# zfountas/deep-active-inference-mc

Measured on AMD Instinct MI355X. Metric: EFE rollouts/sec (64x64 dSprites, 10 MC-samples, depth 5), higher is better.
Workload: dtype f32; 1 GPU; calculate_G_repeated: 128 rows (32 roots x 4 actions) x depth 5 x 10 MC samples per GPU (BASELINE configs[1]) + action posterior; rows_per_gpu=128, samples=10, depth=5, parallelism=episodes sharded x1, weights replicated

## Files before the change

deep-active-inference-mc_amd/build.py:

```python
import hashlib
import os
import subprocess
import sys

HERE = os.path.dirname(os.path.abspath(__file__))
SOURCES = ['csrc/kernels.hip', 'csrc/decoder.hip', 'csrc/encoder.hip', 'csrc/mcts.hip', 'csrc/fused.hip', 'csrc/generic.hip', 'csrc/generic_dec.hip', 'csrc/generic_enc.hip', 'csrc/bf16x3.hip', 'csrc/loss.hip', 'csrc/engine.hip']
HEADERS = ['csrc/kernels.h', 'csrc/philox.h', 'csrc/mfma_pipe.h', 'csrc/ctx_registry.h', '../include/efe_engine.h']
LIB = os.path.join(HERE, 'libefe_mi355x.so')
OPS_SOURCES = ['csrc/torch_ops.cpp']
OPS_LIB = os.path.join(HERE, 'libefe_torch_ops.so')
FLAGS = ['--offload-arch=gfx950', '-O3', '-std=c++17', '-shared', '-fPIC', '-Wno-pass-failed', '-Wl,-soname,libefe_mi355x.so']


def source_digest(files=None):
    h = hashlib.sha256()
    for f in (files or SOURCES + HEADERS):
        path = os.path.join(HERE, f)
        if not os.path.exists(path):
            continue
        h.update(f.encode())
        with open(path, 'rb') as fh:
            h.update(fh.read())
    h.update(' '.join(FLAGS).encode())
    return h.hexdigest()[:16]


def _stamp(lib, marker):
    if not os.path.exists(lib):
        return None
    try:
        data = open(lib, 'rb').read()
        key = (marker + '=').encode()
        i = data.find(key)
        return data[i + len(key):i + len(key) + 16].decode() if i >= 0 else None
    except Exception:
        return None


def needs_build():
    return _stamp(LIB, 'EFE_BUILD_ID') != source_digest()


def _compile_objects(hipcc, srcs, verbose):
    from concurrent.futures import ThreadPoolExecutor
    obj_dir = os.path.join(HERE, 'build')
    os.makedirs(obj_dir, exist_ok=True)
    hdr = source_digest(HEADERS)

    def one(src):
        h = hashlib.sha256(open(src, 'rb').read() + hdr.encode() + ' '.join(FLAGS).encode()).hexdigest()[:16]
        obj = os.path.join(obj_dir, os.path.basename(src) + '.' + h + '.o')
        if not os.path.exists(obj):
            for old in os.listdir(obj_dir):
                if old.startswith(os.path.basename(src) + '.'):
                    os.unlink(os.path.join(obj_dir, old))
            cmd = [hipcc, *[f for f in FLAGS if f != '-shared' and not f.startswith('-Wl,')], '-c', src, '-o', obj]
            if verbose:
                print(' '.join(cmd), flush=True)
            r = subprocess.run(cmd, capture_output=True, text=True)
            if r.returncode != 0:
                sys.stderr.write(r.stdout + r.stderr)
                raise RuntimeError(f'hipcc failed compiling {src}')
        return obj
    with ThreadPoolExecutor(max_workers=min(8, len(srcs))) as ex:
        return list(ex.map(one, srcs))


def build(force=False, verbose=False):
    if force or needs_build():
        hipcc = os.environ.get('HIPCC', '/opt/rocm/bin/hipcc')
        srcs = [os.path.join(HERE, s) for s in SOURCES if os.path.exists(os.path.join(HERE, s))]
        if force:
            import shutil
            shutil.rmtree(os.path.join(HERE, 'build'), ignore_errors=True)
        objs = _compile_objects(hipcc, srcs, verbose)
        stamp = os.path.join(HERE, 'build', 'build_id.cpp')
        with open(stamp, 'w') as fh:
            fh.write('extern "C" const char* efe_build_id(void) {\n'
                     f'    static const char stamp[] = "EFE_BUILD_ID={source_digest()}";      // the marker lets build.py read the stamp from the file without dlopen\n'
                     '    return stamp + 13;\n}\n')
        stamp_o = stamp[:-4] + '.o'
        r = subprocess.run(['g++', '-O1', '-fPIC', '-c', stamp, '-o', stamp_o], capture_output=True, text=True)
        if r.returncode != 0:
            sys.stderr.write(r.stdout + r.stderr)
            raise RuntimeError('g++ failed compiling the build-id stamp')
        cmd = [hipcc, *FLAGS, stamp_o, *objs, '-o', LIB]
        if verbose:
            print(' '.join(cmd))
        r = subprocess.run(cmd, capture_output=True, text=True)
        if r.returncode != 0:
            sys.stderr.write(r.stdout + r.stderr)
            raise RuntimeError('hipcc failed linking libefe_mi355x.so')
    build_torch_ops(force=force, verbose=verbose)
    return LIB


def ops_digest():
    return source_digest(OPS_SOURCES + ['../include/efe_engine.h'])


def build_torch_ops(force=False, verbose=False):
    src = os.path.join(HERE, OPS_SOURCES[0])
    if not os.path.exists(src):
        return None
    if not force and _stamp(OPS_LIB, 'EFE_OPS_BUILD_ID') == ops_digest():
        return OPS_LIB
    import torch
    from torch.utils import cpp_extension as ce
    inc = [f'-I{p}' for p in ce.include_paths()] + ['-I/opt/rocm/include', f'-I{os.path.join(HERE, "..", "include")}']
    tlib = os.path.join(os.path.dirname(torch.__file__), 'lib')
    abi = int(getattr(torch._C, '_GLIBCXX_USE_CXX11_ABI', 1))
    cmd = ['g++', '-O2', '-std=c++17', '-shared', '-fPIC', '-D__HIP_PLATFORM_AMD__=1', '-DUSE_ROCM=1', f'-D_GLIBCXX_USE_CXX11_ABI={abi}',
           f'-DEFE_OPS_BUILD_ID="{ops_digest()}"', *inc, src, '-o', OPS_LIB,
           f'-L{HERE}', '-lefe_mi355x', f'-L{tlib}', '-ltorch', '-ltorch_cpu', '-lc10', '-ltorch_hip', '-lc10_hip',
           '-L/opt/rocm/lib', '-lamdhip64', '-Wl,-rpath,$ORIGIN', f'-Wl,-rpath,{tlib}', '-Wl,-rpath,/opt/rocm/lib']
    if verbose:
        print(' '.join(cmd))
    r = subprocess.run(cmd, capture_output=True, text=True)
    if r.returncode != 0:
        sys.stderr.write(r.stdout + r.stderr)
        raise RuntimeError('g++ failed building libefe_torch_ops.so')
    return OPS_LIB


if __name__ == '__main__':
    print(build(force='--force' in sys.argv, verbose=True))
```

deep-active-inference-mc_amd/csrc/decoder.hip:

```cpp
#include <utility>
#include "mfma_pipe.h"

namespace efe {

template <class F, int... I> __device__ __forceinline__ void static_for_(F&& f, std::integer_sequence<int, I...>) { (f(std::integral_constant<int, I>{}), ...); }
template <int N, class F> __device__ __forceinline__ void static_for(F&& f) { static_for_(f, std::make_integer_sequence<int, N>{}); }

__host__ __device__ constexpr int w3_nch(int G) { return G == 4 ? 5 : 4; }
__host__ __device__ constexpr int w3_prod(int G, int c) {
    return G < 4 ? 5 * ((G >> 1) + 2 * (c >> 1)) + (G & 1) + 2 * (c & 1)
         : G == 4 ? (c < 2 ? 5 * (1 + 2 * c) + 4 : c < 4 ? 20 + 1 + 2 * (c - 2) : 24)
                  : (c < 2 ? 5 * (2 * c) + 4 : 20 + 2 * (c - 2));
}
__host__ __device__ constexpr bool w3_direct(int pp) { return f22_o1(pp / 5) < 0 && f22_o1(pp % 5) < 0; }
__host__ __device__ constexpr int w3_view(int pp) { return 3 * f22_view(pp / 5) + f22_view(pp % 5); }
__host__ __device__ constexpr int w3_mat(int pp) { return 4 * f22_wt(pp / 5) + f22_wt(pp % 5); }
__host__ __device__ constexpr bool w3_hits(int pp, int o) {
    const int r = o >> 2, c = o & 3, pr = pp / 5, pc = pp % 5;
    return (r == f22_o0(pr) || r == f22_o1(pr)) && (c == f22_o0(pc) || c == f22_o1(pc));
}
__host__ __device__ constexpr bool w3_seen(int G, int c, int o) {
    for (int g = 0; g < G; ++g)
        for (int k = 0; k < w3_nch(g); ++k) if (w3_hits(w3_prod(g, k), o)) return true;
    if (!w3_direct(w3_prod(G, c)))
        for (int k = 0; k < w3_nch(G); ++k)
            if ((w3_direct(w3_prod(G, k)) || k < c) && w3_hits(w3_prod(G, k), o)) return true;
    return false;
}
__host__ __device__ constexpr bool w3_uses_view(int G, int vi) {
    for (int k = 0; k < w3_nch(G); ++k) if (w3_view(w3_prod(G, k)) == vi) return true;
    return false;
}
__host__ __device__ constexpr bool f22_in(int a, int r) { return a == 0 ? r <= 1 : (a == 1 ? r == 1 : r >= 1); }
__host__ __device__ constexpr bool w3_reads(int G, int r, int c) {
    for (int vi = 0; vi < 9; ++vi) if (w3_uses_view(G, vi) && f22_in(vi / 3, r) && f22_in(vi % 3, c)) return true;
    return false;
}

constexpr int DA_PS = 17;
constexpr int DA_BIAS = 273 * DA_PS;

__host__ __device__ constexpr int wino_i0(int a) { return a == 0 ? 0 : (a == 2 ? 2 : 1); }
__host__ __device__ constexpr int wino_i1(int a) { return a == 0 ? 2 : (a == 1 ? 2 : (a == 2 ? 1 : 3)); }
__host__ __device__ constexpr float wino_s1(int a) { return a == 1 ? 1.0f : -1.0f; }
__host__ __device__ constexpr float wino_at(int r, int a) { return r == 0 ? (a < 3 ? 1.0f : 0.0f) : (a == 0 ? 0.0f : (a == 1 ? 1.0f : -1.0f)); }

template <int NR, int R0, class Pix>
__device__ __forceinline__ void wino_l1(f32x16 (&out)[NR][2], const float4* __restrict__ U, const float4* sm, const int h,
                                        const int mt_, Pix pix) {
    constexpr int PD = 4;
    const unsigned ln = (threadIdx.x & 63u) * 16u;
    const __amdgpu_buffer_rsrc_t ur = wrsrc(U);
    int mt = mt_; asm volatile("" : "+s"(mt));
    constexpr int a_lo = NR == 2 ? 0 : R0, a_hi = NR == 2 ? 4 : R0 + 3;
    auto ufrag = [&](int a, int b, int kc) { return wfrag(ur, ln, (size_t)(((4 * a + b) * 2 + mt) * 8 + kc) * 64); };
    auto bases = [&](int a, int b, int (&pb)[4]) {
        const int i0 = wino_i0(a), i1 = wino_i1(a), j0 = wino_i0(b), j1 = wino_i1(b);
        pb[0] = pix(i0, j0); pb[1] = pix(i0, j1); pb[2] = pix(i1, j0); pb[3] = pix(i1, j1);
    };
    float4 aq[PD], raw[4];
    int pb[4];
#pragma unroll
    for (int p = 0; p < PD; ++p) aq[p] = ufrag(a_lo, 0, p);
    bases(a_lo, 0, pb);
#pragma unroll
    for (int q = 0; q < 4; ++q) raw[q] = sm[pb[q] + h];
    f32x16 xacc;
    const f32x16 zero = {};
    auto otrans = [&](int a, int b, const f32x16& m, auto mask) {
        constexpr int MASK = decltype(mask)::value;
#pragma unroll
        for (int r = 0; r < NR; ++r) {
            if (!((MASK >> r) & 1)) continue;
            const float car = wino_at(R0 + r, a);
#pragma unroll
            for (int c = 0; c < 2; ++c) {
                const float cbc = wino_at(c, b);
                if (cbc == 0.0f) continue;
                const float cf = car * cbc;
#pragma unroll
                for (int e = 0; e < 16; ++e) out[r][c][e] = __builtin_fmaf(cf, m[e], out[r][c][e]);
            }
        }
    };
    auto xi_row = [&](int a, auto mask) {
        const float s1 = wino_s1(a);
        const int an = a + 1 < a_hi ? a + 1 : a;
#pragma unroll
        for (int b = 0; b < 4; ++b) {
            const float t1 = wino_s1(b);
#pragma unroll
            for (int kc = 0; kc < 8; ++kc) {
                const float4 av = aq[kc % PD];
                aq[kc % PD] = (b * 8 + kc + PD < 32) ? ufrag(a, (b * 8 + kc + PD) >> 3, (kc + PD) & 7) : ufrag(an, 0, (kc + PD) & 7);
                float4 v;
                {
                    const float4 c0 = make_float4(__builtin_fmaf(s1, raw[2].x, raw[0].x), __builtin_fmaf(s1, raw[2].y, raw[0].y),
                                                  __builtin_fmaf(s1, raw[2].z, raw[0].z), __builtin_fmaf(s1, raw[2].w, raw[0].w));
                    const float4 c1 = make_float4(__builtin_fmaf(s1, raw[3].x, raw[1].x), __builtin_fmaf(s1, raw[3].y, raw[1].y),
                                                  __builtin_fmaf(s1, raw[3].z, raw[1].z), __builtin_fmaf(s1, raw[3].w, raw[1].w));
                    v = make_float4(__builtin_fmaf(t1, c1.x, c0.x), __builtin_fmaf(t1, c1.y, c0.y), __builtin_fmaf(t1, c1.z, c0.z), __builtin_fmaf(t1, c1.w, c0.w));
                }
                if (kc < 7) {
#pragma unroll
                    for (int q = 0; q < 4; ++q) raw[q] = sm[pb[q] + 2 * (kc + 1) + h];
                } else {
                    if (b < 3) bases(a, b + 1, pb);
                    else bases(an, 0, pb);
#pragma unroll
                    for (int q = 0; q < 4; ++q) raw[q] = sm[pb[q] + h];
                }
                __builtin_amdgcn_sched_barrier(0);
                f32x16& x = xacc;
                x = __builtin_amdgcn_mfma_f32_32x32x2f32(av.x, v.x, kc == 0 ? zero : x, 0, 0, 0);
                x = __builtin_amdgcn_mfma_f32_32x32x2f32(av.y, v.y, x, 0, 0, 0);
                x = __builtin_amdgcn_mfma_f32_32x32x2f32(av.z, v.z, x, 0, 0, 0);
                x = __builtin_amdgcn_mfma_f32_32x32x2f32(av.w, v.w, x, 0, 0, 0);
            }
            otrans(a, b, xacc, mask);
        }
    };
    if constexpr (NR == 2) {
        xi_row(0, std::integral_constant<int, 1>{});
#pragma unroll 1
        for (int a = 1; a < 3; ++a) xi_row(a, std::integral_constant<int, 3>{});
        xi_row(3, std::integral_constant<int, 2>{});
    } else {
#pragma unroll 1
        for (int a = a_lo; a < a_hi; ++a) xi_row(a, std::integral_constant<int, 1>{});
    }
}
struct F22Nb { int xb, c2[3], r2; };
__device__ __forceinline__ f32x4 f22_wfrag(const __amdgpu_buffer_rsrc_t wr, const unsigned ln, int ct, int m, int kc) {
    return __builtin_bit_cast(f32x4, wfrag(wr, ln + (unsigned)kc * 1024u, (size_t)(m * 4 + ct) * 256));
}
constexpr int F22_PD = 2;
__device__ __forceinline__ void f22_l2_first(f32x4 (&aq)[F22_PD][5], const __amdgpu_buffer_rsrc_t wr, const int dn, const unsigned ln) {
    static_for<F22_PD>([&](auto p) {
        static_for<w3_nch(p >> 2)>([&](auto c) { aq[p][c] = f22_wfrag(wr, ln, dn, w3_mat(w3_prod(p >> 2, c)), p & 3); });
    });
}
__device__ __forceinline__ void f22_l2(f32x4 (&acc)[16], f32x4 (&aq)[F22_PD][5], const __amdgpu_buffer_rsrc_t wr, const int dn,
                                       const unsigned ln, const f32x4 bias4, const f32x4* smv, const F22Nb& nb) {
    constexpr int NST = 24;
    auto px = [&](int i, int jj, int kc) -> f32x4 {
        return smv[(jj == 2 ? nb.c2[i] : (i == 2 ? nb.r2 + jj * DA_PS : nb.xb + (16 * i + jj) * DA_PS)) + 4 * kc];
    };
    auto view = [&](const f32x4 (&x)[9], int vi) -> f32x4 {
        const int va = vi / 3, vb = vi % 3;
        auto cv = [&](int i) -> f32x4 { return vb == 0 ? x[3 * i] - x[3 * i + 1] : (vb == 1 ? x[3 * i + 1] : x[3 * i + 2] - x[3 * i + 1]); };
        return va == 0 ? cv(0) - cv(1) : (va == 1 ? cv(1) : cv(2) - cv(1));
    };
    const f32x4 zero4 = {};
    f32x4 tq[5], xr[9];
    static_for<9>([&](auto i) { if constexpr (w3_reads(0, i / 3, i % 3)) xr[i] = px(i / 3, i % 3, 0); });
    static_for<NST>([&](auto stc) {
        constexpr int ST = decltype(stc)::value, G = ST >> 2, KC = ST & 3, GN = (ST + 1) >> 2, KN = (ST + 1) & 3;
        constexpr int SP = (ST + F22_PD) % NST, GP = SP >> 2, KP = SP & 3;
        f32x4 vw[9], ac[5];
        static_for<9>([&](auto vi) { if constexpr (w3_uses_view(G, vi)) vw[vi] = view(xr, vi); });
#pragma unroll
        for (int c = 0; c < 5; ++c) ac[c] = aq[ST % F22_PD][c];
        static_for<w3_nch(GP)>([&](auto c) { aq[ST % F22_PD][c] = f22_wfrag(wr, ln, ST + F22_PD < NST ? 0 : dn, w3_mat(w3_prod(GP, c)), KP); });
        if constexpr (ST + 1 < NST)
            static_for<9>([&](auto i) { if constexpr (w3_reads(GN, i / 3, i % 3)) xr[i] = px(i / 3, i % 3, KN); });
        __builtin_amdgcn_sched_barrier(0);
#pragma unroll
        for (int e = 0; e < 4; ++e)
            static_for<w3_nch(G)>([&](auto c) {
                constexpr int PP = w3_prod(G, c);
                const float b = vw[w3_view(PP)][e], av = ac[c][e];
                if constexpr (w3_direct(PP)) {
                    constexpr int O = 4 * f22_o0(PP / 5) + f22_o0(PP % 5);
                    constexpr bool FIRST = KC == 0 && !w3_seen(G, c, O);
                    acc[O] = __builtin_amdgcn_mfma_f32_16x16x4f32(av, b, (FIRST && e == 0) ? bias4 : acc[O], 0, 0, 0);
                } else {
                    tq[c] = __builtin_amdgcn_mfma_f32_16x16x4f32(av, b, (KC == 0 && e == 0) ? zero4 : tq[c], 0, 0, 0);
                }
            });
        if constexpr (KC == 3)
            static_for<w3_nch(G)>([&](auto c) {
                constexpr int PP = w3_prod(G, c);
                if constexpr (!w3_direct(PP))
                    static_for<16>([&](auto o) {
                        if constexpr (w3_hits(PP, o)) {
                            if constexpr (w3_seen(G, c, o)) acc[o] = acc[o] + tq[c];
                            else acc[o] = bias4 + tq[c];
                        }
                    });
            });
    });
}
__device__ __forceinline__ void f22_l2_store(f32x4 (&acc)[16], const __amdgpu_buffer_rsrc_t yr, const unsigned yoff, const int ct, const bool on) {
#pragma unroll
    for (int orow = 0; orow < 4; ++orow)
#pragma unroll
        for (int c = 0; c < 2; ++c) {
            u32x4 lo, hi;
#pragma unroll
            for (int e = 0; e < 4; ++e) {
                const unsigned x0 = __builtin_bit_cast(unsigned, relu_bits(acc[4 * orow + c][e]));
                const unsigned x1 = __builtin_bit_cast(unsigned, relu_bits(acc[4 * orow + c + 2][e]));
                const auto sw = __builtin_amdgcn_permlane32_swap(x0, x1, false, false);
                lo[e] = sw[0]; hi[e] = sw[1];
            }
            const unsigned so = (unsigned)(((2 * (orow & 1) + c) * 4096 + 2 * ct * 512 + (orow >> 1) * 32) * 16);
            if (on) {
                __builtin_amdgcn_raw_buffer_store_b128(lo, yr, yoff, so, 0);
                __builtin_amdgcn_raw_buffer_store_b128(hi, yr, yoff, so + 512u * 16u, 0);
            }
        }
}

__global__ void __launch_bounds__(256, 2) k_dec_a(const DecAArgs a) {
    constexpr int NTHR = 256;
    constexpr int NPH = 2048 / NTHR;
    constexpr int NPE = 8;
    extern __shared__ __attribute__((aligned(16))) float4 sm[];
    const int tid = threadIdx.x;
    const int lane = tid & 63;
    const int w = __builtin_amdgcn_readfirstlane(tid >> 6);

    const float4* W1 = reinterpret_cast<const float4*>(a.w1);
    const float4* W2 = reinterpret_cast<const float4*>(a.w2);

    if ((int)blockIdx.x >= a.rows) return;
    int* const slot = reinterpret_cast<int*>(sm + DA_BIAS + 32);
    if (tid == 0) slot[0] = 2 * (int)gridDim.x + atomicAdd(a.queue, 1);
    int nimg = (int)blockIdx.x + (int)gridDim.x;
    f32x4 pf[2 * NPH];
    f32x4* smv = reinterpret_cast<f32x4*>(sm);
    {
        const f32x4* X = reinterpret_cast<const f32x4*>(a.x4) + (size_t)blockIdx.x * 4096;
#pragma unroll
        for (int it = 0; it < 2 * NPH; ++it) pf[it] = X[w * 1024 + it * 64 + lane];
    }
    for (int i = tid; i < 17 * DA_PS; i += NTHR) sm[256 * DA_PS + i] = make_float4(0.f, 0.f, 0.f, 0.f);
    if (tid < 16) sm[DA_BIAS + tid] = reinterpret_cast<const float4*>(a.b1)[tid];
    else if (tid < 32) sm[DA_BIAS + tid] = reinterpret_cast<const float4*>(a.b2)[tid - 16];

    for (int img = blockIdx.x; img < a.rows;) {
        int tl_ = tid; asm volatile("" : "+v"(tl_));
        const int j = tl_ & 31, h = (tl_ >> 5) & 1;
        const bool live = row_live(a.live, img);
        if (live) {
            const int sbase = (64 * w + ((tl_ >> 4) & 3)) * DA_PS + (tl_ & 15);
#pragma unroll
            for (int it = 0; it < 2 * NPH; ++it) smv[sbase + it * 4 * DA_PS] = pf[it];
        }
        __syncthreads();
        const int nnimg = slot[0];
        int ticket = 0;
        if (tid == 0) ticket = 2 * (int)gridDim.x + atomicAdd(a.queue, 1);
        const int l1mt = w >> 1, l1n = 32 * (w & 1) + j;
        const int l1y = 2 * (l1n >> 3) - 1, l1x = 2 * (l1n & 7) - 1;
        if (live) {
            f32x16 l1o[2][2];
#pragma unroll
            for (int g4 = 0; g4 < 4; ++g4) {
                const float4 bb = sm[DA_BIAS + l1mt * 8 + 2 * g4 + h];
#pragma unroll
                for (int rc = 0; rc < 4; ++rc) { l1o[rc >> 1][rc & 1][4 * g4] = bb.x; l1o[rc >> 1][rc & 1][4 * g4 + 1] = bb.y; l1o[rc >> 1][rc & 1][4 * g4 + 2] = bb.z; l1o[rc >> 1][rc & 1][4 * g4 + 3] = bb.w; }
            }
            wino_l1<2, 0>(l1o, W1, sm, h, l1mt, [&](int i, int jj) {
                const int y = l1y + i, x = l1x + jj;
                return ((unsigned)y < 16u && (unsigned)x < 16u ? y * 16 + x : 256) * DA_PS;
            });
            __syncthreads();
            if (tid == 0) slot[0] = ticket;
#pragma unroll
            for (int rc = 0; rc < 4; ++rc) {
                const int pix = (l1y + 1 + (rc >> 1)) * 16 + l1x + 1 + (rc & 1);
#pragma unroll
                for (int g4 = 0; g4 < 4; ++g4) {
// ... 81 lines not shown
    if (tid < 16) sin[DAS_IN * DA_PS + tid] = make_float4(0.f, 0.f, 0.f, 0.f);
    if (tid < 2 * DA_PS) sl1[DAS_L1 * DA_PS + tid] = make_float4(0.f, 0.f, 0.f, 0.f);
    if (tid < 16) sm[DAS_BIAS + tid] = reinterpret_cast<const float4*>(a.b1)[tid];
    else if (tid < 32) sm[DAS_BIAS + tid] = reinterpret_cast<const float4*>(a.b2)[tid - 16];
    __syncthreads();
    const int mt = w >> 1;
    {
        const int r = w & 1, n = j & 15;
        const int ly = 2 * (n >> 3) - 1, lx = 2 * (n & 7) - 1;
        f32x16 o[1][2];
#pragma unroll
        for (int g4 = 0; g4 < 4; ++g4) {
            const float4 bb = sm[DAS_BIAS + mt * 8 + 2 * g4 + h];
#pragma unroll
            for (int c = 0; c < 2; ++c) { o[0][c][4 * g4] = bb.x; o[0][c][4 * g4 + 1] = bb.y; o[0][c][4 * g4 + 2] = bb.z; o[0][c][4 * g4 + 3] = bb.w; }
        }
        auto pix = [&](int i, int jj) {
            const int sy = ly + 1 + i, x = lx + jj, y = 2 * p - 1 + sy;
            return ((unsigned)y < 16u && (unsigned)x < 16u ? sy * 16 + x : DAS_IN) * DA_PS;
        };
        if (r) wino_l1<1, 1>(o, W1, sin, h, mt, pix);
        else wino_l1<1, 0>(o, W1, sin, h, mt, pix);
        if (j < 16)
#pragma unroll
        for (int c = 0; c < 2; ++c)
#pragma unroll
            for (int g4 = 0; g4 < 4; ++g4) {
                float4 v;
                v.x = relu_bits(o[0][c][4 * g4 + 0]); v.y = relu_bits(o[0][c][4 * g4 + 1]);
                v.z = relu_bits(o[0][c][4 * g4 + 2]); v.w = relu_bits(o[0][c][4 * g4 + 3]);
                sl1[((ly + 1 + r) * 16 + lx + 1 + c) * DA_PS + mt * 8 + 2 * g4 + h] = v;
            }
    }
    __syncthreads();
    {
        const int n = lane & 15, g = lane >> 4, bv = n & 7;
        const int zq = DAS_L1 * DA_PS + g;
        F22Nb nb;
        nb.xb = 2 * bv * DA_PS + g;
        nb.c2[0] = bv == 7 ? zq : nb.xb + 2 * DA_PS;
        nb.c2[1] = bv == 7 ? zq : nb.xb + 18 * DA_PS;
        nb.c2[2] = (bv == 7 || p == 7) ? zq : nb.xb + 34 * DA_PS;
        nb.r2 = p == 7 ? zq : nb.xb + 32 * DA_PS;
        const unsigned ln = (unsigned)lane * 16u;
        const unsigned yoff = (unsigned)(((32 * p + 2 * bv + (g >> 1)) * 2 + (g & 1)) * 16);
        const __amdgpu_buffer_rsrc_t yr = wrsrc(a.y2 + (size_t)img * (32 * 32 * 64));
        const __amdgpu_buffer_rsrc_t wr = wrsrc(W2 + w * 256);
        f32x4 aq[F22_PD][5], acc2[16];
        f22_l2_first(aq, wr, 0, ln);
        const f32x4 bias4 = reinterpret_cast<const f32x4*>(sm)[DAS_BIAS + 16 + 4 * w + g];
        f22_l2(acc2, aq, wr, 0, ln, bias4, reinterpret_cast<const f32x4*>(sl1), nb);
        f22_l2_store(acc2, yr, yoff, w, n < 8);
    }
}

constexpr size_t DA_LDS_BYTES = (DA_BIAS + 33) * sizeof(float4);
int init_dec_b_kernels();
int init_decoder_kernels() {
    if (hipFuncSetAttribute((const void*)k_dec_a, hipFuncAttributeMaxDynamicSharedMemorySize, DA_LDS_BYTES) != hipSuccess) return 1;
    if (hipFuncSetAttribute((const void*)k_dec_a_s, hipFuncAttributeMaxDynamicSharedMemorySize, DAS_LDS_BYTES) != hipSuccess) return 1;
    return init_dec_b_kernels();
}

void launch_dec_a(const DecAArgs& a, hipStream_t st) {
    if (a.parts == 8) {
        hipLaunchKernelGGL(k_dec_a_s, dim3(a.rows * 8), dim3(256), DAS_LDS_BYTES, st, a);
        return;
    }
    const size_t lds = DA_LDS_BYTES;
    const int grid = a.rows < 512 ? a.rows : 512;
    hipLaunchKernelGGL(k_dec_a, dim3(grid), dim3(256), lds, st, a);
}


template <int PARTS>
__global__ void __launch_bounds__(256, 2) k_dec_b4(const DecBArgs a) {
    constexpr int SR = 4, NW = 4, NTHR = 256;
    constexpr int DB_RP = 33;
    constexpr int DB_PS = 17;
    constexpr int DB_IN_F4 = (SR + 1) * DB_RP * DB_PS;
    constexpr int DB_YROWS = 4 * SR + 2;
    constexpr int NPF = (SR + 1) * 512 / NTHR;
    constexpr int NS = 32 / SR;
    constexpr int NST = 24;
    extern __shared__ __attribute__((aligned(16))) float4 sm[];
    float* sH = reinterpret_cast<float*>(sm + DB_IN_F4);
    __shared__ float4 sb3[8];
    const int tid = threadIdx.x;
    const int lane = tid & 63;
    const int w = __builtin_amdgcn_readfirstlane(tid >> 6);
    const int g = lane >> 4, v = lane & 15;
    const int u = w >> 1, hf = w & 1;
    constexpr int parts = PARTS;
    const int img = parts == 1 ? (int)blockIdx.x : (int)(blockIdx.x >> 2);
    const int qtr = parts == 1 ? 0 : (int)(blockIdx.x & 3);
    if (!row_live(a.live, img)) return;
    const int s_lo = parts == 1 ? 0 : (qtr ? 2 * qtr - 1 : 0);
    const int s_hi = parts == 1 ? NS : 2 * qtr + 2;

    const int mg = a.m0 + img;
    const int gi = mg / a.rows_per_group;
    const int r = mg - gi * a.rows_per_group;
    int gt, gp, gs;
    group_decode(a.gm, gi, gt, gp, gs);
    const int mode = (gp == 0 && a.reward0) ? 1 : 0;
    const int slot = (gp == 0 && a.store0) ? gt * a.gm.S + gs : -1;
    float* po = (slot >= 0) ? a.po + ((size_t)slot * a.rows_per_group + r) * 4096 : nullptr;

    __shared__ float sq[4 * NTHR];
    __shared__ float sQ[4];
    if (tid < 8) sb3[tid] = reinterpret_cast<const float4*>(a.b3)[tid];
    if (tid < (SR + 1) * 16) sm[((tid >> 4) * DB_RP + 32) * DB_PS + (tid & 15)] = make_float4(0.f, 0.f, 0.f, 0.f);
    f32x4 w4a;
    {
        const int kh = v >> 2, kw = v & 3;
#pragma unroll
        for (int rr = 0; rr < 4; ++rr) w4a[rr] = (kh < 3 && kw < 3) ? a.w4[(3 * kh + kw) * 32 + 16 * hf + 4 * g + rr] : 0.f;
    }

    const float4* X = reinterpret_cast<const float4*>(a.y2) + (size_t)img * (32 * 32 * 16);
    const __amdgpu_buffer_rsrc_t wr = wrsrc(a.w3 + (size_t)hf * 4 * 64 * 4);
    const unsigned ln = (unsigned)lane * 16u;
    auto wf = [&](int m, int kc) -> f32x4 { return __builtin_bit_cast(f32x4, wfrag(wr, ln, (size_t)(m * 8 + kc) * 64)); };
    const float D1 = 1.00001f, D0 = 0.00001f;
    float part = 0.f;
    f32x4 pf[NPF];
    f32x4* smv = reinterpret_cast<f32x4*>(sm);
    const f32x4* Xv = reinterpret_cast<const f32x4*>(X);
    auto y2_at = [&](int iy, int idx) -> size_t { return (size_t)(((iy & 1) * 16 + ((idx & 511) >> 5)) * 512 + (iy >> 1) * 32 + (idx & 31)); };
#pragma unroll
    for (int it = 0; it < NPF; ++it) { const int idx = it * NTHR + tid; pf[it] = Xv[y2_at(min(SR * s_lo + (idx >> 9), 31), idx)]; }

    const int xb = (2 * u * DB_RP + 2 * v) * DB_PS + g;
    auto px = [&](int i, int jj, int kc) -> f32x4 { return smv[xb + (i * DB_RP + jj) * DB_PS + 4 * kc]; };
    auto view = [&](const f32x4 (&x)[9], int vi) -> f32x4 {
        const int va = vi / 3, vb = vi % 3;
        auto cv = [&](int i) -> f32x4 { return vb == 0 ? x[3 * i] - x[3 * i + 1] : (vb == 1 ? x[3 * i + 1] : x[3 * i + 2] - x[3 * i + 1]); };
        return va == 0 ? cv(0) - cv(1) : (va == 1 ? cv(1) : cv(2) - cv(1));
    };

    constexpr int RWG = 2 * SR / NW;
    float gh[RWG][6], gpr[RWG];
    auto g_load = [&](int oh, int q, int r0y, int hb0) {
#pragma unroll
        for (int kh = 0; kh < 3; ++kh) {
            const int tr = oh + 1 - kh;
            const bool rv = tr >= 0 && tr <= 63;
            int hs = hb0 + (tr - r0y);
            hs = hs < 0 ? hs + DB_YROWS : hs;
            hs = hs >= DB_YROWS ? hs - DB_YROWS : hs;
            hs = rv ? hs : 0;
            const float* hq = sH + ((hs * 2) * 3 + kh) * 64 + lane;
            gh[q][2 * kh] = hq[0]; gh[q][2 * kh + 1] = hq[3 * 64];
        }
    };
    auto g_sig = [&](int oh, int q) {
        float val = a.b4;
#pragma unroll
        for (int kh = 0; kh < 3; ++kh) {
            const int tr = oh + 1 - kh;
            val += (tr >= 0 && tr <= 63) ? gh[q][2 * kh] + gh[q][2 * kh + 1] : 0.f;
        }
        gpr[q] = hw_sigmoid(val);
    };
    auto g_term = [&](int oh, int q) {
#pragma clang fp contract(off)
        const float pr = gpr[q];
        const float l1 = hw_log(D1 - pr), l0 = hw_log(D0 + pr);
        const float te = __builtin_fmaf(pr - 1.0f, l1, -(pr * l0));
        const float tw = reward_term(pr, oh, lane, 64, 64, a.reward_intent);
        const float t = mode == 0 ? te : tw;
        part += oh >= 0 ? t : 0.0f;
    };
    auto g_store = [&](int oh, int q) {
        if (po && oh >= 0) {
            int owl = lane; asm volatile("" : "+v"(owl));
            (po + oh * 64)[owl] = gpr[q];
        }
    };
    auto prefetch = [&](int sn, int tl) {
#pragma unroll
        for (int it = 0; it < NPF; ++it) {
            const int idx = it * NTHR + tl;
            const int grow = min(SR * sn + (idx >> 9), 31);
            pf[it] = Xv[y2_at(grow, idx)];
        }
    };

    auto fold = [&](int k) { sq[k * NTHR + tid] = part; part = 0.f; };
    int hb = 0, hbp = 0;
    for (int s = s_lo; s < s_hi; ++s) {
        int tl = tid; asm volatile("" : "+v"(tl));
        const bool gq = parts == 1 ? true : s == 2 * qtr + 1;
        const int oh0 = 2 * SR * (s - 1) - 1 + w, oh1 = oh0 + NW;
#pragma unroll
        for (int it = 0; it < NPF; ++it) {
            const int idx = it * NTHR + tl;
            const int rl = idx >> 9, seg = (idx & 511) >> 5, wi = idx & 31;
            const int ix = 2 * (wi >> 1) + (seg >> 3), c4 = 2 * (seg & 7) + (wi & 1);
            smv[(rl * DB_RP + ix) * DB_PS + c4] = (SR * s + rl < 32) ? pf[it] : (f32x4)(0.f);
        }
        f32x4 aq[5];
#pragma unroll
        for (int c = 0; c < w3_nch(0); ++c) aq[c] = wf(w3_mat(w3_prod(0, c)), 0);
        __syncthreads();

        const f32x4 bias4 = __builtin_bit_cast(f32x4, sb3[4 * hf + g]);
        const f32x4 zero4 = {};
        f32x4 acc[16], tq[5];
        f32x4 xr[9];
        static_for<9>([&](auto i) { if constexpr (w3_reads(0, i / 3, i % 3)) xr[i] = px(i / 3, i % 3, 0); });
        static_for<NST>([&](auto stc) {
            constexpr int ST = decltype(stc)::value, G = ST >> 2, KC = ST & 3, GN = (ST + 1) >> 2, KN = (ST + 1) & 3;
            f32x4 vw[9], ac[5];
            static_for<9>([&](auto vi) { if constexpr (w3_uses_view(G, vi)) vw[vi] = view(xr, vi); });
#pragma unroll
            for (int c = 0; c < 5; ++c) ac[c] = aq[c];
            if constexpr (ST + 1 < NST) {
                static_for<w3_nch(GN)>([&](auto c) { aq[c] = wf(w3_mat(w3_prod(GN, c)), KN); });
                static_for<9>([&](auto i) { if constexpr (w3_reads(GN, i / 3, i % 3)) xr[i] = px(i / 3, i % 3, KN); });
            }
            __builtin_amdgcn_sched_barrier(0);
#pragma unroll
            for (int e = 0; e < 4; ++e)
                static_for<w3_nch(G)>([&](auto c) {
                    constexpr int PP = w3_prod(G, c);
                    const float b = vw[w3_view(PP)][e], av = ac[c][e];
                    if constexpr (w3_direct(PP)) {
                        constexpr int O = 4 * f22_o0(PP / 5) + f22_o0(PP % 5);
                        constexpr bool FIRST = KC == 0 && !w3_seen(G, c, O);
                        acc[O] = __builtin_amdgcn_mfma_f32_16x16x4f32(av, b, (FIRST && e == 0) ? bias4 : acc[O], 0, 0, 0);
                    } else {
                        tq[c] = __builtin_amdgcn_mfma_f32_16x16x4f32(av, b, (KC == 0 && e == 0) ? zero4 : tq[c], 0, 0, 0);
                    }
                });
            if constexpr (KC == 3)
                static_for<w3_nch(G)>([&](auto c) {
                    constexpr int PP = w3_prod(G, c);
                    if constexpr (!w3_direct(PP))
                        static_for<16>([&](auto o) {
                            if constexpr (w3_hits(PP, o)) {
                                if constexpr (w3_seen(G, c, o)) acc[o] = acc[o] + tq[c];
                                else acc[o] = bias4 + tq[c];
                            }
                        });
                });
            if (gq) {
                if constexpr (ST == 0) { g_load(oh0, 0, 2 * SR * (s - 1), hbp); g_load(oh1, 1, 2 * SR * (s - 1), hbp); }
                if constexpr (ST == 2) g_sig(oh0, 0);
                if constexpr (ST == 5) g_term(oh0, 0);
                if constexpr (ST == 8) g_sig(oh1, 1);
                if constexpr (ST == 11) g_term(oh1, 1);
            }
        });
        prefetch((s < NS - 1) ? s + 1 : NS - 1, tl);
#pragma unroll
        for (int orow = 0; orow < 4; ++orow) {
            f32x4 T[4];
#pragma unroll
            for (int oc = 0; oc < 4; ++oc)
#pragma unroll
                for (int e = 0; e < 4; ++e) acc[4 * orow + oc][e] = relu_bits(acc[4 * orow + oc][e]);
#pragma unroll
            for (int e = 0; e < 4; ++e)
#pragma unroll
                for (int oc = 0; oc < 4; ++oc)
                    T[oc] = __builtin_amdgcn_mfma_f32_16x16x4f32(w4a[e], acc[4 * orow + oc][e], e == 0 ? zero4 : T[oc], 0, 0, 0);
            f32x4 hv;
            hv[0] = (T[1][0] + T[0][1]) + dpp_shr1_zero(T[3][2]);
            hv[1] = (T[2][0] + T[1][1]) + T[0][2];
            hv[2] = (T[3][0] + T[2][1]) + T[1][2];
            hv[3] = (dpp_shl1_zero(T[0][0]) + T[3][1]) + T[2][2];
            int hsw = hb + 4 * u + orow;
            hsw = hsw >= DB_YROWS ? hsw - DB_YROWS : hsw;
            if (g < 3) *reinterpret_cast<f32x4*>(sH + ((hsw * 2 + hf) * 3 + g) * 64 + 4 * v) = hv;
        }
        __syncthreads();
        if (gq) { g_store(oh0, 0); g_store(oh1, 1); }
        if (parts == 1 && (s == 2 || s == 4 || s == 6)) fold(s / 2 - 1);
        if (s == s_hi - 1) {
#pragma unroll
            for (int q = 0; q <= RWG; ++q) {
                if (q == RWG && (w != 0 || s != NS - 1)) break;
                const int oh = 2 * SR * s - 1 + q * NW + w;
                g_load(oh, 0, 2 * SR * s, hb); g_sig(oh, 0); g_term(oh, 0); g_store(oh, 0);
            }
        }
        hbp = hb;
        hb += 2 * SR;
        hb = hb >= DB_YROWS ? hb - DB_YROWS : hb;
    }
    fold(parts == 1 ? 3 : 0);
    __syncthreads();
    if (w < (parts == 1 ? 4 : 1)) {
        const float* qk = sq + w * NTHR + lane;
        float val = (qk[0] + qk[64]) + (qk[128] + qk[192]);
#pragma unroll
        for (int o = 32; o > 0; o >>= 1) val += __shfl_xor(val, o);
        if (lane == 0) sQ[w] = val;
    }
    __syncthreads();
    if (tid == 0) {
        if (parts == 1) a.val[mg] = (sQ[0] + sQ[1]) + (sQ[2] + sQ[3]);
        else a.valq[(size_t)mg * 4 + qtr] = sQ[0];
    }
}

constexpr size_t DB_LDS4D = ((5 * 33) * 17) * sizeof(float4) + 18 * 2 * 3 * 64 * sizeof(float);
int init_dec_b_kernels() {
    if (hipFuncSetAttribute((const void*)k_dec_b4<1>, hipFuncAttributeMaxDynamicSharedMemorySize, DB_LDS4D) != hipSuccess) return 1;
    if (hipFuncSetAttribute((const void*)k_dec_b4<4>, hipFuncAttributeMaxDynamicSharedMemorySize, DB_LDS4D) != hipSuccess) return 1;
    return 0;
}

void launch_dec_b(const DecBArgs& a, hipStream_t st) {
    if (a.parts == 4) hipLaunchKernelGGL(k_dec_b4<4>, dim3(a.rows * 4), dim3(256), DB_LDS4D, st, a);
    else hipLaunchKernelGGL(k_dec_b4<1>, dim3(a.rows), dim3(256), DB_LDS4D, st, a);
}

__host__ __device__ inline int fc4_spg(int mtiles) { return ((mtiles + 7) / 8 + 7) / 8; }
template <int NT>
__global__ void __launch_bounds__(256, 2) k_fc4(const GemmArgs a) {
    constexpr int RT = 32 * NT;
    extern __shared__ __attribute__((aligned(16))) float4 sm[];
    const int tid = threadIdx.x;
    const int lane = tid & 63;
    const int w = __builtin_amdgcn_readfirstlane(tid >> 6);
    const int j = lane & 31, h = lane >> 5;
    const int fgrp = blockIdx.x & 7;
    const int nper = gridDim.x >> 3, k = blockIdx.x >> 3;
    const int SPG = fc4_spg(a.mtiles);
    const int nsteps = ((a.n_pix + RT - 1) / RT) * SPG;
    const int q0 = (int)(((long)nsteps * k) / nper), q1 = (int)(((long)nsteps * (k + 1)) / nper);
    f32x4* smv = reinterpret_cast<f32x4*>(sm);
    const float4* Wl = reinterpret_cast<const float4*>(a.Wp);
    auto xaddr = [&](int t, int (&bs)[NT], int (&sw)[NT], int& wt) {
        wt = t;
// ... 83 lines not shown
```

Baseline: 11630 rollouts/s.

## Share a software-pipelined Winograd contraction between decoder layers with scalar view forming

Factors the F(2x2) Winograd-style contraction used by two decoder layers into one shared routine, f22_contract. It forms the transformed input views per MFMA k-element as scalars interleaved with the MFMAs under sched_group_barrier. It double-buffers the input registers, defers adding the temporaries into the accumulators into the next group's first step, and reuses middle-row view halves from earlier groups so group 5 skips some LDS reads. It also drops weight prefetch depth from 2 to 1, simplifies the index math for staging the prefetched input, and disables packed-fp32 ops for decoder.hip via a per-file compiler flag. The aim is to hide VALU view construction and LDS loads behind MFMA work and cut register pressure, at the cost of much more intricate scheduling that depends on the compiler honoring the hints.

```diff
diff --git a/deep-active-inference-mc_amd/build.py b/deep-active-inference-mc_amd/build.py
--- a/deep-active-inference-mc_amd/build.py
+++ b/deep-active-inference-mc_amd/build.py
@@ -10,6 +10,7 @@
 OPS_SOURCES = ['csrc/torch_ops.cpp']
 OPS_LIB = os.path.join(HERE, 'libefe_torch_ops.so')
 FLAGS = ['--offload-arch=gfx950', '-O3', '-std=c++17', '-shared', '-fPIC', '-Wno-pass-failed', '-Wl,-soname,libefe_mi355x.so']
+EXTRA_FLAGS = {'csrc/decoder.hip': ['-Xclang', '-target-feature', '-Xclang', '-packed-fp32-ops']}
 
 
 def source_digest(files=None):
@@ -22,6 +23,8 @@
         with open(path, 'rb') as fh:
             h.update(fh.read())
     h.update(' '.join(FLAGS).encode())
+    for f in sorted(EXTRA_FLAGS):
+        h.update((f + ' ' + ' '.join(EXTRA_FLAGS[f])).encode())
     return h.hexdigest()[:16]
 
 
@@ -48,13 +51,14 @@
     hdr = source_digest(HEADERS)
 
     def one(src):
-        h = hashlib.sha256(open(src, 'rb').read() + hdr.encode() + ' '.join(FLAGS).encode()).hexdigest()[:16]
+        extra = EXTRA_FLAGS.get(os.path.relpath(src, HERE).replace(os.sep, '/'), [])
+        h = hashlib.sha256(open(src, 'rb').read() + hdr.encode() + ' '.join(FLAGS + extra).encode()).hexdigest()[:16]
         obj = os.path.join(obj_dir, os.path.basename(src) + '.' + h + '.o')
         if not os.path.exists(obj):
             for old in os.listdir(obj_dir):
                 if old.startswith(os.path.basename(src) + '.'):
                     os.unlink(os.path.join(obj_dir, old))
-            cmd = [hipcc, *[f for f in FLAGS if f != '-shared' and not f.startswith('-Wl,')], '-c', src, '-o', obj]
+            cmd = [hipcc, *[f for f in FLAGS if f != '-shared' and not f.startswith('-Wl,')], *extra, '-c', src, '-o', obj]
             if verbose:
                 print(' '.join(cmd), flush=True)
             r = subprocess.run(cmd, capture_output=True, text=True)
diff --git a/deep-active-inference-mc_amd/csrc/decoder.hip b/deep-active-inference-mc_amd/csrc/decoder.hip
--- a/deep-active-inference-mc_amd/csrc/decoder.hip
+++ b/deep-active-inference-mc_amd/csrc/decoder.hip
@@ -32,9 +32,114 @@
     return false;
 }
 __host__ __device__ constexpr bool f22_in(int a, int r) { return a == 0 ? r <= 1 : (a == 1 ? r == 1 : r >= 1); }
+__host__ __device__ constexpr bool w3_only_views(int G, int v0, int v1) {
+    for (int vi = 0; vi < 9; ++vi) if (w3_uses_view(G, vi) != (vi == v0 || vi == v1)) return false;
+    return true;
+}
+static_assert(w3_only_views(2, 3, -1) && w3_uses_view(4, 5) && w3_only_views(5, 2, 6),
+              "group 5's views (0, 2) and (2, 0) take their middle-row halves from the views (1, 0) of group 2 and (1, 2) of group 4, which run before it");
 __host__ __device__ constexpr bool w3_reads(int G, int r, int c) {
+    if (G == 5 && r == 1) return false;
     for (int vi = 0; vi < 9; ++vi) if (w3_uses_view(G, vi) && f22_in(vi / 3, r) && f22_in(vi % 3, c)) return true;
     return false;
+}
+
+__host__ __device__ constexpr bool w3_has_tmp(int G) {
+    for (int k = 0; k < w3_nch(G); ++k) if (!w3_direct(w3_prod(G, k))) return true;
+    return false;
+}
+static_assert(!w3_has_tmp(5), "a group's temporaries are added under the NEXT group's first step (f22_contract): the last group must have none");
+__host__ __device__ constexpr bool w3_direct_out(int G, int o) {
+    for (int k = 0; k < w3_nch(G); ++k)
+        if (w3_direct(w3_prod(G, k)) && 4 * f22_o0(w3_prod(G, k) / 5) + f22_o0(w3_prod(G, k) % 5) == o) return true;
+    return false;
+}
+template <int VB> __device__ __forceinline__ float f22_cv(const f32x4 (&x)[9], const int i, const int e) {
+    return VB == 0 ? x[3 * i][e] - x[3 * i + 1][e] : (VB == 1 ? x[3 * i + 1][e] : x[3 * i + 2][e] - x[3 * i + 1][e]);
+}
+constexpr int F22_NST = 24;
+constexpr int F22_VPG = 5;
+template <int PD, class Px, class Wf, class Piece>
+__device__ __forceinline__ void f22_contract(f32x4 (&acc)[16], f32x4 (&aq)[PD][5], const f32x4 bias4, Px px, Wf wf, Piece piece) {
+    const f32x4 zero4 = {};
+    f32x4 tq[5], tp[5], xr[2][9];
+    float vc[9], vn[9], vm[9];
+    static_for<9>([&](auto i) { if constexpr (w3_reads(0, i / 3, i % 3)) xr[0][i] = px(i / 3, i % 3, 0); });
+    f32x4 k10[4], k12[4];
+    auto form = [&](float (&dst)[9], const f32x4 (&x)[9], auto g, auto kc, const int e) {
+        constexpr int FG = decltype(g)::value, FK = decltype(kc)::value;
+        static_for<9>([&](auto vi) {
+            if constexpr (w3_uses_view(FG, vi)) {
+                constexpr int va = vi / 3, vb = vi % 3;
+                float c1;
+                if constexpr (FG == 5) c1 = vb == 2 ? k12[FK][e] : k10[FK][e];
+                else if constexpr (FG == 4 && vi == 8) c1 = dst[5];
+                else c1 = f22_cv<vb>(x, 1, e);
+                if constexpr (va == 1) dst[vi] = c1;
+                else dst[vi] = f22_cv<vb>(x, va, e) - c1;
+                if constexpr (vi != 4) asm volatile("" : "+v"(dst[vi]));
+                if constexpr (FG == 2) k10[FK][e] = dst[vi];
+                if constexpr (FG == 4 && vi == 5) k12[FK][e] = dst[vi];
+            }
+        });
+    };
+    form(vc, xr[0], std::integral_constant<int, 0>{}, std::integral_constant<int, 0>{}, 0);
+    static_for<F22_NST>([&](auto stc) {
+        constexpr int ST = decltype(stc)::value, G = ST >> 2, KC = ST & 3, GN = (ST + 1) >> 2, KN = (ST + 1) & 3;
+        constexpr int CUR = ST & 1, NXT = CUR ^ 1;
+        f32x4 ac[5];
+#pragma unroll
+        for (int c = 0; c < 5; ++c) ac[c] = aq[ST % PD][c];
+        wf(aq[ST % PD], std::integral_constant<int, ST + PD>{});
+        __builtin_amdgcn_sched_barrier(0);
+        static_for<4>([&](auto ec) {
+            constexpr int E = decltype(ec)::value;
+            if constexpr (E == 2 && ST + 1 < F22_NST)
+                static_for<9>([&](auto i) { if constexpr (w3_reads(GN, i / 3, i % 3)) xr[NXT][i] = px(i / 3, i % 3, KN); });
+            if constexpr (KC == 0 && G > 0 && w3_has_tmp(G > 0 ? G - 1 : 0)) {
+                constexpr int GP = G > 0 ? G - 1 : 0;
+                static_for<w3_nch(GP)>([&](auto c) {
+                    constexpr int PP = w3_prod(GP, c);
+                    if constexpr (!w3_direct(PP))
+                        static_for<16>([&](auto o) {
+                            if constexpr (w3_hits(PP, o) && (w3_direct_out(G, o) ? 0 : (c < 3 ? (int)c : 3)) == E) {
+                                if constexpr (w3_seen(GP, c, o)) acc[o] = acc[o] + tp[c];
+                                else acc[o] = bias4 + tp[c];
+                            }
+                        });
+                });
+            }
+            constexpr std::integral_constant<int, G> gc{};
+            constexpr std::integral_constant<int, KC> kcc{};
+            if constexpr (E == 0) form(vn, xr[CUR], gc, kcc, 1);
+            if constexpr (E == 1) { form(vn, xr[CUR], gc, kcc, 2); form(vm, xr[CUR], gc, kcc, 3); }
+            if constexpr (E == 2) piece(std::integral_constant<int, ST>{});
+            if constexpr (E == 3 && ST + 1 < F22_NST) form(vn, xr[NXT], std::integral_constant<int, GN < 6 ? GN : 0>{}, std::integral_constant<int, KN>{}, 0);
+            static_for<w3_nch(G)>([&](auto c) {
+                constexpr int PP = w3_prod(G, c);
+                const float b = vc[w3_view(PP)], av = ac[c][E];
+                if constexpr (w3_direct(PP)) {
+                    constexpr int O = 4 * f22_o0(PP / 5) + f22_o0(PP % 5);
+                    constexpr bool FIRST = KC == 0 && !w3_seen(G, c, O);
+                    acc[O] = __builtin_amdgcn_mfma_f32_16x16x4f32(av, b, (FIRST && E == 0) ? bias4 : acc[O], 0, 0, 0);
+                } else {
+                    tq[c] = __builtin_amdgcn_mfma_f32_16x16x4f32(av, b, (KC == 0 && E == 0) ? zero4 : tq[c], 0, 0, 0);
+                }
+            });
+            if constexpr (E == 2) __builtin_amdgcn_sched_group_barrier(0x100, 9, 0);
+            static_for<w3_nch(G)>([&](auto c) {
+                if constexpr (E != 3 || c >= 2) __builtin_amdgcn_sched_group_barrier(0x002, F22_VPG, 0);
+                __builtin_amdgcn_sched_group_barrier(0x008, 1, 0);
+            });
+            __builtin_amdgcn_sched_barrier(0);
+            static_for<9>([&](auto vi) {
+                if constexpr (E == 3 ? (ST + 1 < F22_NST && w3_uses_view(GN < 6 ? GN : 0, vi)) : w3_uses_view(G, vi)) vc[vi] = E == 2 ? vm[vi] : vn[vi];
+            });
+        });
+        if constexpr (KC == 3)
+#pragma unroll
+            for (int c = 0; c < 5; ++c) tp[c] = tq[c];
+    });
 }
 
 constexpr int DA_PS = 17;
@@ -134,7 +239,7 @@
 __device__ __forceinline__ f32x4 f22_wfrag(const __amdgpu_buffer_rsrc_t wr, const unsigned ln, int ct, int m, int kc) {
     return __builtin_bit_cast(f32x4, wfrag(wr, ln + (unsigned)kc * 1024u, (size_t)(m * 4 + ct) * 256));
 }
-constexpr int F22_PD = 2;
+constexpr int F22_PD = 1;
 __device__ __forceinline__ void f22_l2_first(f32x4 (&aq)[F22_PD][5], const __amdgpu_buffer_rsrc_t wr, const int dn, const unsigned ln) {
     static_for<F22_PD>([&](auto p) {
         static_for<w3_nch(p >> 2)>([&](auto c) { aq[p][c] = f22_wfrag(wr, ln, dn, w3_mat(w3_prod(p >> 2, c)), p & 3); });
@@ -142,54 +247,15 @@
 }
 __device__ __forceinline__ void f22_l2(f32x4 (&acc)[16], f32x4 (&aq)[F22_PD][5], const __amdgpu_buffer_rsrc_t wr, const int dn,
                                        const unsigned ln, const f32x4 bias4, const f32x4* smv, const F22Nb& nb) {
-    constexpr int NST = 24;
-    auto px = [&](int i, int jj, int kc) -> f32x4 {
-        return smv[(jj == 2 ? nb.c2[i] : (i == 2 ? nb.r2 + jj * DA_PS : nb.xb + (16 * i + jj) * DA_PS)) + 4 * kc];
-    };
-    auto view = [&](const f32x4 (&x)[9], int vi) -> f32x4 {
-        const int va = vi / 3, vb = vi % 3;
-        auto cv = [&](int i) -> f32x4 { return vb == 0 ? x[3 * i] - x[3 * i + 1] : (vb == 1 ? x[3 * i + 1] : x[3 * i + 2] - x[3 * i + 1]); };
-        return va == 0 ? cv(0) - cv(1) : (va == 1 ? cv(1) : cv(2) - cv(1));
-    };
-    const f32x4 zero4 = {};
-    f32x4 tq[5], xr[9];
-    static_for<9>([&](auto i) { if constexpr (w3_reads(0, i / 3, i % 3)) xr[i] = px(i / 3, i % 3, 0); });
-    static_for<NST>([&](auto stc) {
-        constexpr int ST = decltype(stc)::value, G = ST >> 2, KC = ST & 3, GN = (ST + 1) >> 2, KN = (ST + 1) & 3;
-        constexpr int SP = (ST + F22_PD) % NST, GP = SP >> 2, KP = SP & 3;
-        f32x4 vw[9], ac[5];
-        static_for<9>([&](auto vi) { if constexpr (w3_uses_view(G, vi)) vw[vi] = view(xr, vi); });
-#pragma unroll
-        for (int c = 0; c < 5; ++c) ac[c] = aq[ST % F22_PD][c];
-        static_for<w3_nch(GP)>([&](auto c) { aq[ST % F22_PD][c] = f22_wfrag(wr, ln, ST + F22_PD < NST ? 0 : dn, w3_mat(w3_prod(GP, c)), KP); });
-        if constexpr (ST + 1 < NST)
-            static_for<9>([&](auto i) { if constexpr (w3_reads(GN, i / 3, i % 3)) xr[i] = px(i / 3, i % 3, KN); });
-        __builtin_amdgcn_sched_barrier(0);
-#pragma unroll
-        for (int e = 0; e < 4; ++e)
-            static_for<w3_nch(G)>([&](auto c) {
-                constexpr int PP = w3_prod(G, c);
-                const float b = vw[w3_view(PP)][e], av = ac[c][e];
-                if constexpr (w3_direct(PP)) {
-                    constexpr int O = 4 * f22_o0(PP / 5) + f22_o0(PP % 5);
-                    constexpr bool FIRST = KC == 0 && !w3_seen(G, c, O);
-                    acc[O] = __builtin_amdgcn_mfma_f32_16x16x4f32(av, b, (FIRST && e == 0) ? bias4 : acc[O], 0, 0, 0);
-                } else {
-                    tq[c] = __builtin_amdgcn_mfma_f32_16x16x4f32(av, b, (KC == 0 && e == 0) ? zero4 : tq[c], 0, 0, 0);
-                }
-            });
-        if constexpr (KC == 3)
-            static_for<w3_nch(G)>([&](auto c) {
-                constexpr int PP = w3_prod(G, c);
-                if constexpr (!w3_direct(PP))
-                    static_for<16>([&](auto o) {
-                        if constexpr (w3_hits(PP, o)) {
-                            if constexpr (w3_seen(G, c, o)) acc[o] = acc[o] + tq[c];
-                            else acc[o] = bias4 + tq[c];
-                        }
-                    });
-            });
-    });
+    f22_contract<F22_PD>(acc, aq, bias4,
+        [&](int i, int jj, int kc) -> f32x4 {
+            return smv[(jj == 2 ? nb.c2[i] : (i == 2 ? nb.r2 + jj * DA_PS : nb.xb + (16 * i + jj) * DA_PS)) + 4 * kc];
+        },
+        [&](f32x4 (&dst)[5], auto spc) {
+            constexpr int SP = decltype(spc)::value % F22_NST, GP = SP >> 2, KP = SP & 3;
+            static_for<w3_nch(GP)>([&](auto c) { dst[c] = f22_wfrag(wr, ln, decltype(spc)::value < F22_NST ? 0 : dn, w3_mat(w3_prod(GP, c)), KP); });
+        },
+        [](auto) {});
 }
 __device__ __forceinline__ void f22_l2_store(f32x4 (&acc)[16], const __amdgpu_buffer_rsrc_t yr, const unsigned yoff, const int ct, const bool on) {
 #pragma unroll
@@ -437,7 +503,6 @@
     constexpr int DB_YROWS = 4 * SR + 2;
     constexpr int NPF = (SR + 1) * 512 / NTHR;
     constexpr int NS = 32 / SR;
-    constexpr int NST = 24;
     extern __shared__ __attribute__((aligned(16))) float4 sm[];
     float* sH = reinterpret_cast<float*>(sm + DB_IN_F4);
     __shared__ float4 sb3[8];
@@ -482,18 +547,13 @@
     f32x4 pf[NPF];
     f32x4* smv = reinterpret_cast<f32x4*>(sm);
     const f32x4* Xv = reinterpret_cast<const f32x4*>(X);
-    auto y2_at = [&](int iy, int idx) -> size_t { return (size_t)(((iy & 1) * 16 + ((idx & 511) >> 5)) * 512 + (iy >> 1) * 32 + (idx & 31)); };
-#pragma unroll
-    for (int it = 0; it < NPF; ++it) { const int idx = it * NTHR + tid; pf[it] = Xv[y2_at(min(SR * s_lo + (idx >> 9), 31), idx)]; }
+    static_assert(NTHR == 256, "the row / segment split of a staged float4 below (it >> 1, 8 (it & 1) + (t >> 5)) is that of 256 threads and 512-float4 rows");
+    auto y2_at = [&](int iy, int it, int t) -> size_t { return (size_t)(((iy & 1) * 16 + 8 * (it & 1)) * 512 + (iy >> 1) * 32) + (size_t)((t >> 5) * 512 + (t & 31)); };
+#pragma unroll
+    for (int it = 0; it < NPF; ++it) pf[it] = Xv[y2_at(min(SR * s_lo + (it >> 1), 31), it, tid)];
 
     const int xb = (2 * u * DB_RP + 2 * v) * DB_PS + g;
     auto px = [&](int i, int jj, int kc) -> f32x4 { return smv[xb + (i * DB_RP + jj) * DB_PS + 4 * kc]; };
-    auto view = [&](const f32x4 (&x)[9], int vi) -> f32x4 {
-        const int va = vi / 3, vb = vi % 3;
-        auto cv = [&](int i) -> f32x4 { return vb == 0 ? x[3 * i] - x[3 * i + 1] : (vb == 1 ? x[3 * i + 1] : x[3 * i + 2] - x[3 * i + 1]); };
-        return va == 0 ? cv(0) - cv(1) : (va == 1 ? cv(1) : cv(2) - cv(1));
-    };
-
     constexpr int RWG = 2 * SR / NW;
     float gh[RWG][6], gpr[RWG];
     auto g_load = [&](int oh, int q, int r0y, int hb0) {
@@ -535,11 +595,7 @@
     };
     auto prefetch = [&](int sn, int tl) {
 #pragma unroll
-        for (int it = 0; it < NPF; ++it) {
-            const int idx = it * NTHR + tl;
-            const int grow = min(SR * sn + (idx >> 9), 31);
-            pf[it] = Xv[y2_at(grow, idx)];
-        }
+        for (int it = 0; it < NPF; ++it) pf[it] = Xv[y2_at(min(SR * sn + (it >> 1), 31), it, tl)];
     };
 
     auto fold = [&](int k) { sq[k * NTHR + tid] = part; part = 0.f; };
@@ -550,64 +606,33 @@
         const int oh0 = 2 * SR * (s - 1) - 1 + w, oh1 = oh0 + NW;
 #pragma unroll
         for (int it = 0; it < NPF; ++it) {
-            const int idx = it * NTHR + tl;
-            const int rl = idx >> 9, seg = (idx & 511) >> 5, wi = idx & 31;
-            const int ix = 2 * (wi >> 1) + (seg >> 3), c4 = 2 * (seg & 7) + (wi & 1);
+            const int rl = it >> 1, wi = tl & 31;
+            const int ix = 2 * (wi >> 1) + (it & 1), c4 = 2 * (tl >> 5) + (wi & 1);
             smv[(rl * DB_RP + ix) * DB_PS + c4] = (SR * s + rl < 32) ? pf[it] : (f32x4)(0.f);
         }
-        f32x4 aq[5];
-#pragma unroll
-        for (int c = 0; c < w3_nch(0); ++c) aq[c] = wf(w3_mat(w3_prod(0, c)), 0);
+        f32x4 aq[1][5];
+#pragma unroll
+        for (int c = 0; c < w3_nch(0); ++c) aq[0][c] = wf(w3_mat(w3_prod(0, c)), 0);
         __syncthreads();
 
         const f32x4 bias4 = __builtin_bit_cast(f32x4, sb3[4 * hf + g]);
         const f32x4 zero4 = {};
-        f32x4 acc[16], tq[5];
-        f32x4 xr[9];
-        static_for<9>([&](auto i) { if constexpr (w3_reads(0, i / 3, i % 3)) xr[i] = px(i / 3, i % 3, 0); });
-        static_for<NST>([&](auto stc) {
-            constexpr int ST = decltype(stc)::value, G = ST >> 2, KC = ST & 3, GN = (ST + 1) >> 2, KN = (ST + 1) & 3;
-            f32x4 vw[9], ac[5];
-            static_for<9>([&](auto vi) { if constexpr (w3_uses_view(G, vi)) vw[vi] = view(xr, vi); });
-#pragma unroll
-            for (int c = 0; c < 5; ++c) ac[c] = aq[c];
-            if constexpr (ST + 1 < NST) {
-                static_for<w3_nch(GN)>([&](auto c) { aq[c] = wf(w3_mat(w3_prod(GN, c)), KN); });
-                static_for<9>([&](auto i) { if constexpr (w3_reads(GN, i / 3, i % 3)) xr[i] = px(i / 3, i % 3, KN); });
-            }
-            __builtin_amdgcn_sched_barrier(0);
-#pragma unroll
-            for (int e = 0; e < 4; ++e)
-                static_for<w3_nch(G)>([&](auto c) {
-                    constexpr int PP = w3_prod(G, c);
-                    const float b = vw[w3_view(PP)][e], av = ac[c][e];
-                    if constexpr (w3_direct(PP)) {
-                        constexpr int O = 4 * f22_o0(PP / 5) + f22_o0(PP % 5);
-                        constexpr bool FIRST = KC == 0 && !w3_seen(G, c, O);
-                        acc[O] = __builtin_amdgcn_mfma_f32_16x16x4f32(av, b, (FIRST && e == 0) ? bias4 : acc[O], 0, 0, 0);
-                    } else {
-                        tq[c] = __builtin_amdgcn_mfma_f32_16x16x4f32(av, b, (KC == 0 && e == 0) ? zero4 : tq[c], 0, 0, 0);
-                    }
-                });
-            if constexpr (KC == 3)
-                static_for<w3_nch(G)>([&](auto c) {
-                    constexpr int PP = w3_prod(G, c);
-                    if constexpr (!w3_direct(PP))
-                        static_for<16>([&](auto o) {
-                            if constexpr (w3_hits(PP, o)) {
-                                if constexpr (w3_seen(G, c, o)) acc[o] = acc[o] + tq[c];
-                                else acc[o] = bias4 + tq[c];
-                            }
-                        });
-                });
-            if (gq) {
-                if constexpr (ST == 0) { g_load(oh0, 0, 2 * SR * (s - 1), hbp); g_load(oh1, 1, 2 * SR * (s - 1), hbp); }
-                if constexpr (ST == 2) g_sig(oh0, 0);
-                if constexpr (ST == 5) g_term(oh0, 0);
-                if constexpr (ST == 8) g_sig(oh1, 1);
-                if constexpr (ST == 11) g_term(oh1, 1);
-            }
-        });
+        f32x4 acc[16];
+        f22_contract<1>(acc, aq, bias4, px,
+            [&](f32x4 (&dst)[5], auto spc) {
+                constexpr int SP = decltype(spc)::value;
+                if constexpr (SP < F22_NST) static_for<w3_nch(SP >> 2)>([&](auto c) { dst[c] = wf(w3_mat(w3_prod(SP >> 2, c)), SP & 3); });
+            },
+            [&](auto stc) {
+                constexpr int ST = decltype(stc)::value;
+                if (gq) {
+                    if constexpr (ST == 0) { g_load(oh0, 0, 2 * SR * (s - 1), hbp); g_load(oh1, 1, 2 * SR * (s - 1), hbp); }
+                    if constexpr (ST == 2) g_sig(oh0, 0);
+                    if constexpr (ST == 5) g_term(oh0, 0);
+                    if constexpr (ST == 8) g_sig(oh1, 1);
+                    if constexpr (ST == 11) g_term(oh1, 1);
+                }
+            });
         prefetch((s < NS - 1) ? s + 1 : NS - 1, tl);
 #pragma unroll
         for (int orow = 0; orow < 4; ++orow) {
```

Measured after the change: 11950 rollouts/s, median of 6. 1.03x the previous value.
